# LiHaoy-ux/DQO-MAP

Measured on AMD Instinct MI355X. Metric: mapping iters/sec (fwd+bwd raster) @ 500k Gaussians 1200×680; PSNR vs ref, higher is better.
Workload: dtype f32; 1 GPU; cfg3: surfel room, ONE map of 500000 Gaussians, 1200x680, 8 object ids, SH degree 3, per-object render (object gate) + per-object masked loss (sum over objects of 0.8 L1 colour + 1.0 depth L1 on the object's own mask) + attach loss, raster fwd+bwd + Adam (6 groups); path=fused (hipGraph replays of 4 iterations each); rccl_ranks=1, backend=none (one rank), list_split=0, list_split_backward=0, graph_unroll=4, sync_mode=lazy, selfcheck=skipped, P=500000, P_visible=196562, view=room, adam=exact-sparse, adam_rows_touched=197735, attach_loss_members=49997

## Files before the change

### dqo-map_amd/_dqo_native.py

```python
import ctypes
import os

_HERE = os.path.dirname(os.path.abspath(__file__))
LIB_PATH = os.path.join(_HERE, "lib", "libdqoraster.so")

c_f = ctypes.c_float
c_i32 = ctypes.c_int32
c_vp = ctypes.c_void_p


class DqoRastParams(ctypes.Structure):
    _fields_ = [("P", c_i32), ("D", c_i32), ("M", c_i32), ("W", c_i32), ("H", c_i32), ("prefiltered", c_i32), ("debug", c_i32),
                ("tanfovx", c_f), ("tanfovy", c_f), ("cx", c_f), ("cy", c_f), ("scale_modifier", c_f), ("color_sigma", c_f),
                ("opaque_threshold", c_f), ("depth_threshold", c_f), ("normal_threshold", c_f), ("T_threshold", c_f)]


class DqoRastInputs(ctypes.Structure):
    _fields_ = [(n, c_vp) for n in ("bg", "means3D", "shs", "colors_precomp", "opacities", "scales", "rotations", "cov3D_precomp",
                                    "viewmatrix", "projmatrix", "campos", "tile_mask", "row_flags")]


class DqoRastOutputs(ctypes.Structure):
    _fields_ = [(n, c_vp) for n in ("out_color", "out_depth", "out_hit_color", "out_hit_depth", "out_hit_color_weight",
                                    "out_hit_depth_weight", "out_T", "n_touched", "radii")]
# ... 27 lines not shown

class DqoRastParamGrads(ctypes.Structure):
    _fields_ = [(n, c_vp) for n in ("dL_dfeatures_dc", "dL_dfeatures_rest", "dL_dopacity_raw", "dL_dscaling_raw", "dL_drotation_raw")]


class DqoRastHeader(ctypes.Structure):
    _fields_ = [("num_rendered", ctypes.c_uint32), ("num_tiles", ctypes.c_uint32), ("overflow", ctypes.c_uint32),
                ("max_tile_count", ctypes.c_uint32), ("num_visible", ctypes.c_uint32), ("num_candidates", ctypes.c_uint32),
                ("stage", ctypes.c_uint32), ("reserved", ctypes.c_uint32)]


class DqoProfileEntry(ctypes.Structure):
    _fields_ = [("name", ctypes.c_char * 48), ("total_ms", ctypes.c_double), ("calls", ctypes.c_uint32)]


class DqoAdamStep(ctypes.Structure):
    _fields_ = ([("P", c_i32), ("M", c_i32), ("step", c_i32), ("beta1", c_f), ("beta2", c_f), ("eps", c_f), ("lr_xyz", c_f),
                 ("lr_f_dc", c_f), ("lr_f_rest", c_f), ("lr_opacity", c_f), ("lr_scaling", c_f), ("lr_rotation", c_f)] +
                [(n, c_vp) for n in ("xyz", "shs", "opacity_raw", "scaling_raw", "rotation_raw", "g_means3D", "g_sh", "g_opacity",
                                     "g_scales", "g_rotations", "m_xyz", "m_shs", "m_opacity", "m_scaling", "m_rotation", "v_xyz",
                                     "v_shs", "v_opacity", "v_scaling", "v_rotation", "act_opacity", "act_scales", "act_rotations", "radii", "step_dev", "moment_live",
                                     "attach_mask", "init_xyz", "init_scaling_raw", "init_rotation_raw")] +
                [("attach_count", c_i32), ("attach_partial", c_vp), ("frame_header", c_vp), ("block_ticket", c_vp), ("bias_table", c_vp), ("attach_gains", c_vp),
                 ("row_flags", c_vp), ("confidence", c_vp), ("lr_table", c_vp)])

ROW_FROZEN, ROW_HIDDEN = 1, 2


class DqoAdamTensor(ctypes.Structure):
    _fields_ = [("p", c_vp), ("g", c_vp), ("m", c_vp), ("v", c_vp), ("n", ctypes.c_int64), ("lr", ctypes.c_double)]


EXPORTS = ("dqo_abi_version", "dqo_abi_sizeof", "dqo_last_error", "dqo_profile_enable", "dqo_profile_collect", "dqo_map_activate",
           "dqo_map_loss_workspace_bytes", "dqo_map_loss_fwd_bwd", "dqo_map_ssim_workspace_bytes", "dqo_map_ssim_fwd_bwd", "dqo_map_adam_step", "dqo_adam_multi_dev", "dqo_map_attach_workspace_bytes",
           "dqo_map_attach_loss_fwd_bwd", "dqo_adam_multi", "dqo_accumulate_gaussian_error", "dqo_accumulate_gaussian_confidence", "dqo_rast_geom_bytes", "dqo_rast_image_bytes",
           "dqo_rast_binning_bytes", "dqo_rast_binning_bytes_bucketed",
           "dqo_rast_backward_workspace_bytes", "dqo_rast_forward_prepare", "dqo_rast_read_header", "dqo_rast_forward_render",
           "dqo_rast_forward", "dqo_rast_forward_async", "dqo_rast_backward", "dqo_rast_backward_adam", "dqo_mark_visible", "dqo_knn3_workspace_bytes", "dqo_knn3",
           "dqo_quadric_iou_fwd_bwd", "dqo_quadric_adam", "dqo_tile_count_mask", "dqo_transmission_mask", "dqo_tile_color_error", "dqo_knn3_query_workspace_bytes",
           "dqo_knn3_query", "dqo_knn3_query_within", "dqo_knn3_query_grouped", "dqo_icp_workspace_bytes", "dqo_icp_normal_equations",
           "dqo_attach_pixels", "dqo_attach_decide", "dqo_growth_scales", "dqo_growth_inside", "dqo_error_maps", "dqo_map_history_merge",
           "dqo_rast_forward_prepare_params", "dqo_rast_forward_render_params", "dqo_rast_forward_async_params", "dqo_rast_backward_params",
           "dqo_icp_gauss_newton", "dqo_track_preprocess_workspace_bytes", "dqo_track_preprocess", "dqo_track_pyramid_pixels",
           "dqo_track_pyramid_workspace_bytes", "dqo_track_pyramid", "dqo_track_fill_model_depth", "dqo_track_p2p_workspace_bytes",
           "dqo_track_p2p_loss")

_lib = None
# ... 133 lines not shown
```

### dqo-map_amd/csrc/dqo_adam.h

```cpp
#pragma once
#include "dqo_common.h"

struct AdamArgs {
    int P, M;
    float beta1, beta2, eps, bc2_sqrt;
    float omb1, omb2;
    double beta1_d, beta2_d;
    float step_xyz, step_dc, step_rest, step_opacity, step_scaling, step_rotation;
    float *xyz, *shs, *opacity_raw, *scaling_raw, *rotation_raw;
    const float *g_xyz, *g_shs, *g_opacity, *g_scales, *g_rot;
    float *m_xyz, *m_shs, *m_opacity, *m_scaling, *m_rotation;
    float *v_xyz, *v_shs, *v_opacity, *v_scaling, *v_rotation;
    float *act_opacity, *act_scales, *act_rotations;
    const int32_t* radii;
    uint64_t row_magic;
    const int32_t* step_dev;
    float lr_xyz, lr_dc, lr_rest, lr_opacity, lr_scaling, lr_rotation;
    const uint8_t* attach_mask;
    const float *init_xyz, *init_scaling, *init_rotation;
    float attach_g3, attach_g4;
    float* attach_partial;
    const DqoRastHeader* frame_header;
    int32_t* step_advance;
    int32_t* block_ticket;
    float* bias_table;
    const float* attach_gains;
    const uint8_t* row_flags;
    float* confidence;
    const float* lr_table;
};

static inline double dqo_beta_double(float b) { return (double)(long long)((double)b * 1e7 + 0.5) / 1e7; }

int dqo_adam_args(const DqoAdamStep* st, int blocks, AdamArgs* out, bool* attach);

#ifdef __HIPCC__
constexpr int ADAM_THREADS = 256;

template <typename T>
__device__ __forceinline__ T ldnt(const T* p) {
    return __builtin_nontemporal_load(p);
}
template <typename T>
__device__ __forceinline__ void stnt(T v, T* p) {
    __builtin_nontemporal_store(v, p);
}

__device__ __forceinline__ float adam_wave_red(float v) {
#pragma unroll
    for (int off = 32; off > 0; off >>= 1) v += __shfl_xor(v, off);
    return v;
}

__device__ __forceinline__ void adam1(float& p, float g, float& m, float& v, const AdamArgs& a, float step_size) {
#pragma clang fp contract(off)
    m = m + (g - m) * a.omb1;
    v = v * a.beta2 + a.omb2 * g * g;
    const float denom = sqrtf(v) / a.bc2_sqrt + a.eps;
    p = p - step_size * (m / denom);
}

struct AdamGradGlobal {
    const AdamArgs& a;
    __device__ __forceinline__ float xyz(int, uint32_t, size_t i, bool has_g) const { return a.g_xyz[has_g ? i : 0]; }
    __device__ __forceinline__ float scales(int, uint32_t, size_t i, bool has_g) const { return a.g_scales[has_g ? i : 0]; }
    __device__ __forceinline__ float sh(int, uint32_t, uint32_t ei, uint32_t e0, bool has_g) const { return ldnt(&a.g_shs[has_g ? ei : e0]); }
    __device__ __forceinline__ float opacity(int, uint32_t i, bool has_g) const { return a.g_opacity[has_g ? i : 0u]; }
    __device__ __forceinline__ float4 rot(int, uint32_t i, bool has_g) const { return reinterpret_cast<const float4*>(a.g_rot)[has_g ? i : 0u]; }
    __device__ __forceinline__ bool dc_nonzero(int, uint32_t i, bool has_g) const {
        const size_t e = has_g ? (size_t)i * (size_t)(3 * a.M) : 0;
        const float g0 = ldnt(&a.g_shs[e]), g1 = ldnt(&a.g_shs[e + 1]), g2 = ldnt(&a.g_shs[e + 2]);
        return has_g && (g0 != 0.f || g1 != 0.f || g2 != 0.f);
    }
};

__device__ __forceinline__ void adam_bias_compute(const AdamArgs& a, const int step, float* out ) {
    const double t = (double)step;
    const double bc1 = 1.0 - pow(a.beta1_d, t), bc2 = 1.0 - pow(a.beta2_d, t);
    out[0] = (float)sqrt(bc2);
    float lr[6] = {a.lr_xyz, a.lr_dc, a.lr_rest, a.lr_opacity, a.lr_scaling, a.lr_rotation};
    if (a.lr_table != nullptr) {
#pragma unroll
// ... 62 lines not shown
    const float4 g = has_g ? x.gr_ld : make_float4(0.f, 0.f, 0.f, 0.f);
    const float nrm = fmaxf(sqrtf(q.x * q.x + q.y * q.y + q.z * q.z + q.w * q.w), 1e-12f);
    const float yx = q.x / nrm, yy = q.y / nrm, yz = q.z / nrm, yw = q.w / nrm;
    const float dot = yx * g.x + yy * g.y + yz * g.z + yw * g.w;
    float4 gq = make_float4((g.x - yx * dot) / nrm, (g.y - yy * dot) / nrm, (g.z - yz * dot) / nrm, (g.w - yw * dot) / nrm);
    if (ATTACH) {
        const bool at = ((r >> 30) & 1u) != 0u;
        const float4 q0 = x.q0;
        const float4 d = at ? make_float4(q.x - q0.x, q.y - q0.y, q.z - q0.z, q.w - q0.w) : make_float4(0.f, 0.f, 0.f, 0.f);
        gq.x += a.attach_g4 * d.x, gq.y += a.attach_g4 * d.y, gq.z += a.attach_g4 * d.z, gq.w += a.attach_g4 * d.w;
        att_sum += 0.5f * a.attach_g4 * (d.x * d.x + d.y * d.y + d.z * d.z + d.w * d.w);
    }
    adam1(q.x, gq.x, mq.x, vq.x, a, a.step_rotation);
    adam1(q.y, gq.y, mq.y, vq.y, a, a.step_rotation);
    adam1(q.z, gq.z, mq.z, vq.z, a, a.step_rotation);
    adam1(q.w, gq.w, mq.w, vq.w, a, a.step_rotation);
    reinterpret_cast<float4*>(a.rotation_raw)[i] = q;
    if (a.act_rotations) {
        const float n2 = fmaxf(sqrtf(q.x * q.x + q.y * q.y + q.z * q.z + q.w * q.w), 1e-12f);
        reinterpret_cast<float4*>(a.act_rotations)[i] = make_float4(q.x / n2, q.y / n2, q.z / n2, q.w / n2);
    }
    reinterpret_cast<float4*>(a.m_rotation)[i] = mq;
    reinterpret_cast<float4*>(a.v_rotation)[i] = vq;
    if (a.confidence != nullptr && x.dc_nz) a.confidence[i] = x.conf + 1.0f;
}

template <bool ATTACH, int THREADS, typename GradSrc>
__device__ __forceinline__ float adam_passes(const AdamArgs& a, const uint32_t* s_rows, const int n_rows, const GradSrc& gsrc) {
    const int tid = threadIdx.x;
    float att_sum = 0.f;
    for (int e = tid; e < 3 * n_rows; e += THREADS) {
        const uint32_t k = (uint32_t)e / 3u, j = (uint32_t)e - 3u * k, r = s_rows[k];
        const bool has_g = (r >> 31) != 0u;
        const size_t i = (size_t)(r & 0x3fffffffu) * 3 + j;
        AdamXyzVals x;
        x.p = a.xyz[i], x.m = a.m_xyz[i], x.v = a.v_xyz[i];
        x.ps = a.scaling_raw[i], x.ms = a.m_scaling[i], x.vs = a.v_scaling[i];
        x.gx_ld = gsrc.xyz((int)k, j, i, has_g), x.gs_ld = gsrc.scales((int)k, j, i, has_g);
        x.p0 = x.ps0 = 0.f;
        if (ATTACH) {
            const size_t ai = ((r >> 30) & 1u) ? i : 0;
            x.p0 = a.init_xyz[ai], x.ps0 = a.init_scaling[ai];
        }
        adam_xyz_update<ATTACH>(a, r, i, x, att_sum);
    }
    const uint32_t row = (uint32_t)a.M * 3u;
// ... 186 lines not shown
```

### dqo-map_amd/csrc/map_fused.hip

```cpp
#include "dqo_adam.h"
#include "dqo_common.h"

namespace {

__global__ __launch_bounds__(256) void activate_kernel(int P, const float* __restrict__ opacity_raw, const float* __restrict__ scaling_raw,
                                                       const float* __restrict__ rotation_raw, float* __restrict__ opacity,
                                                       float* __restrict__ scales, float* __restrict__ rotations) {
    const int i = blockIdx.x * blockDim.x + threadIdx.x;
    if (i >= P) return;
    opacity[i] = 1.0f / (1.0f + expf(-opacity_raw[i]));
#pragma unroll
    for (int k = 0; k < 3; k++) scales[3 * i + k] = expf(scaling_raw[3 * i + k]);
    const float4 q = reinterpret_cast<const float4*>(rotation_raw)[i];
    const float n = fmaxf(sqrtf(q.x * q.x + q.y * q.y + q.z * q.z + q.w * q.w), 1e-12f);
    reinterpret_cast<float4*>(rotations)[i] = make_float4(q.x / n, q.y / n, q.z / n, q.w / n);
}

constexpr int LOSS_THREADS = 256;

__device__ __forceinline__ float wave_red(float v) {
#pragma unroll
    for (int off = 32; off > 0; off >>= 1) v += __shfl_xor(v, off);
    return v;
}
// ... 227 lines not shown
        } else {
            const float th0 = acosf(dot), s_th0 = sinf(th0), tht = th0 * t;
            const float s0 = sinf(th0 - tht) / s_th0, s1 = sinf(tht) / s_th0;
            o = make_float4(s0 * v0.x + s1 * v1.x, s0 * v0.y + s1 * v1.y, s0 * v0.z + s1 * v1.z, s0 * v0.w + s1 * v1.w);
        }
        reinterpret_cast<float4*>(rotation)[i] = o;
    }
    const int row = 3 * M;
    const size_t e0 = (size_t)blockIdx.x * HM_THREADS * row;
    const int n = min(HM_THREADS, P - blockIdx.x * HM_THREADS) * row;
    for (int e = threadIdx.x; e < n; e += HM_THREADS) {
        const int r = blockIdx.x * HM_THREADS + e / row;
        if (row_flags != nullptr && (row_flags[r] & DQO_ROW_FROZEN) != 0u) continue;
        shs[e0 + e] = shs0[e0 + e] * w0 + u0 * shs[e0 + e];
    }
}

__global__ void adam_advance_kernel(int32_t* step_dev, const DqoRastHeader* frame_header) {
    if (frame_header != nullptr && frame_header->overflow != 0u) return;
    *step_dev += 1;
}

template <bool SPARSE, bool ATTACH>
__device__ __forceinline__ void adam_block(AdamArgs a, uint8_t* __restrict__ moment_live);

template <bool SPARSE, bool ATTACH>
__global__ __launch_bounds__(ADAM_THREADS) void adam_kernel(const AdamArgs a, uint8_t* __restrict__ moment_live) {
    if (a.frame_header != nullptr && a.frame_header->overflow != 0u) return;
    adam_block<SPARSE, ATTACH>(a, moment_live);
    adam_take_ticket(a);
}

template <bool SPARSE, bool ATTACH>
__device__ __forceinline__ void adam_block(AdamArgs a, uint8_t* __restrict__ moment_live) {
    __shared__ uint32_t s_rows[ADAM_THREADS];
    __shared__ float s_att[ADAM_THREADS / 64];
    __shared__ int s_wave_n[ADAM_THREADS / 64];
    __shared__ float s_ss[7];
    const int tid = threadIdx.x, lane = tid & 63, wave = tid >> 6;
    if (a.step_dev != nullptr && tid == 0) adam_bias_to_lds(a, s_ss);
    const int idx = blockIdx.x * ADAM_THREADS + tid;
    bool hg = false, act = false, att = false;
    if (idx < a.P && !(a.row_flags != nullptr && (a.row_flags[idx] & DQO_ROW_FROZEN) != 0u)) {
        hg = a.radii == nullptr || a.radii[idx] > 0;
        act = !SPARSE || hg || moment_live[idx] != 0;
        if (SPARSE && hg) moment_live[idx] = 1;
        if (ATTACH) att = a.attach_mask[idx] != 0;
    }
    const unsigned long long am = __builtin_amdgcn_ballot_w64(act);
    if (lane == 0) s_wave_n[wave] = (int)__popcll(am);
    __syncthreads();
    if (a.step_dev != nullptr) adam_bias_from_lds(a, s_ss);
    if (ATTACH) adam_attach_gains(a);
    int before = 0, n_rows = 0;
#pragma unroll
    for (int w = 0; w < ADAM_THREADS / 64; w++) {
        const int c = s_wave_n[w];
        before += w < wave ? c : 0;
        n_rows += c;
    }
    if (act) s_rows[before + (int)__popcll(am & ((1ull << lane) - 1ull))] = (uint32_t)idx | (hg ? 0x80000000u : 0u) | (att ? 0x40000000u : 0u);
    __syncthreads();
    if (n_rows == 0) {
        if (ATTACH && a.attach_partial != nullptr && tid == 0) a.attach_partial[blockIdx.x] = 0.f;
        return;
    }
    float att_sum = adam_passes<ATTACH, ADAM_THREADS>(a, s_rows, n_rows, AdamGradGlobal{a});
    if (ATTACH && a.attach_partial != nullptr) {
        att_sum = wave_red(att_sum);
        if (lane == 0) s_att[wave] = att_sum;
// ... 49 lines not shown
    a.step_xyz = (float)((double)st->lr_xyz / bc1);
    a.step_dc = (float)((double)st->lr_f_dc / bc1);
    a.step_rest = (float)((double)st->lr_f_rest / bc1);
    a.step_opacity = (float)((double)st->lr_opacity / bc1);
    a.step_scaling = (float)((double)st->lr_scaling / bc1);
    a.step_rotation = (float)((double)st->lr_rotation / bc1);
    a.xyz = st->xyz, a.shs = st->shs, a.opacity_raw = st->opacity_raw, a.scaling_raw = st->scaling_raw, a.rotation_raw = st->rotation_raw;
    a.g_xyz = st->g_means3D, a.g_shs = st->g_sh, a.g_opacity = st->g_opacity, a.g_scales = st->g_scales, a.g_rot = st->g_rotations;
    a.m_xyz = st->m_xyz, a.m_shs = st->m_shs, a.m_opacity = st->m_opacity, a.m_scaling = st->m_scaling, a.m_rotation = st->m_rotation;
    a.v_xyz = st->v_xyz, a.v_shs = st->v_shs, a.v_opacity = st->v_opacity, a.v_scaling = st->v_scaling, a.v_rotation = st->v_rotation;
    a.act_opacity = st->act_opacity, a.act_scales = st->act_scales, a.act_rotations = st->act_rotations;
    a.radii = st->radii;
    a.step_dev = st->step_dev;
    a.lr_xyz = st->lr_xyz, a.lr_dc = st->lr_f_dc, a.lr_rest = st->lr_f_rest, a.lr_opacity = st->lr_opacity, a.lr_scaling = st->lr_scaling;
    a.lr_rotation = st->lr_rotation;
    a.attach_mask = st->attach_mask, a.init_xyz = st->init_xyz, a.init_scaling = st->init_scaling_raw, a.init_rotation = st->init_rotation_raw;
    a.attach_partial = st->attach_partial, a.frame_header = st->frame_header;
    const bool advance_inside = st->step_dev != nullptr && st->block_ticket != nullptr && blocks > 0;
    a.step_advance = advance_inside ? st->step_dev : nullptr, a.block_ticket = st->block_ticket;
    a.bias_table = (advance_inside && st->step_dev != nullptr) ? st->bias_table : nullptr;
    const bool attach = st->attach_mask != nullptr && (st->attach_count > 0 || st->attach_gains != nullptr);
    a.attach_gains = attach ? st->attach_gains : nullptr;
    a.row_flags = st->row_flags, a.confidence = st->confidence, a.lr_table = st->lr_table;
    DQO_CHECK_ARG(st->lr_table == nullptr || st->step_dev != nullptr, "lr_table is read on the device: it needs step_dev");
    DQO_CHECK_ARG(!attach || (st->init_xyz && st->init_scaling_raw && st->init_rotation_raw), "attach_mask needs the three init_* tensors");
    DQO_CHECK_ARG(st->P < (1 << 30), "P must stay below 2^30");
    a.attach_g3 = (attach && st->attach_count > 0) ? (float)(2000.0 / (3.0 * (double)st->attach_count)) : 0.f;
    a.attach_g4 = (attach && st->attach_count > 0) ? (float)(2000.0 / (4.0 * (double)st->attach_count)) : 0.f;
    DQO_CHECK_ARG(st->M >= 0 && st->M * 3 < 256, "M out of range");
    a.row_magic = st->M > 0 ? ((1ull << 39) + (uint64_t)(3 * st->M) - 1) / (uint64_t)(3 * st->M) : 0ull;
    DQO_CHECK_ARG((int64_t)st->P * (st->M > 0 ? st->M : 1) * 3 < (int64_t)0x7fffffff, "P * M * 3 must stay below 2^31");
    DQO_CHECK_ARG(st->moment_live == nullptr || st->radii != nullptr, "moment_live needs radii");
    *out = a;
    *attach_out = attach;
    return DQO_OK;
}

int dqo_launch_map_adam(const DqoAdamStep* st, hipStream_t s) {
    const int blocks = (st->P + ADAM_THREADS - 1) / ADAM_THREADS;
    AdamArgs a;
    bool attach = false;
    const int rc = dqo_adam_args(st, blocks, &a, &attach);
    if (rc) return rc;
    const bool advance_inside = a.step_advance != nullptr;
    if (blocks > 0) {
        if (st->moment_live != nullptr) {
            if (attach) DQO_LAUNCH("adam_kernel", (adam_kernel<true, true>), dim3(blocks), dim3(ADAM_THREADS), s, a, st->moment_live);
            else DQO_LAUNCH("adam_kernel", (adam_kernel<true, false>), dim3(blocks), dim3(ADAM_THREADS), s, a, st->moment_live);
        } else {
            if (attach) DQO_LAUNCH("adam_kernel", (adam_kernel<false, true>), dim3(blocks), dim3(ADAM_THREADS), s, a, st->moment_live);
            else DQO_LAUNCH("adam_kernel", (adam_kernel<false, false>), dim3(blocks), dim3(ADAM_THREADS), s, a, st->moment_live);
        }
    }
    if (st->step_dev != nullptr && !advance_inside)
        DQO_LAUNCH("adam_advance_kernel", adam_advance_kernel, dim3(1), dim3(1), s, st->step_dev, st->frame_header);
    return DQO_OK;
}

namespace {
constexpr int ADAMM_THREADS = 256, ADAMM_PER_THREAD = 4;
struct AdamMultiArgs {
    float* p[DQO_ADAM_MULTI_MAX];
    const float* g[DQO_ADAM_MULTI_MAX];
    float* m[DQO_ADAM_MULTI_MAX];
    float* v[DQO_ADAM_MULTI_MAX];
    int64_t n[DQO_ADAM_MULTI_MAX];
    float step_size[DQO_ADAM_MULTI_MAX];
    uint32_t first_block[DQO_ADAM_MULTI_MAX + 1];
    int n_tensors;
    float beta1, beta2, omb1, omb2, eps, bc2_sqrt;
    const int32_t* step_dev;
    double beta1_d, beta2_d;
    double lr[DQO_ADAM_MULTI_MAX];
};
// ... 94 lines not shown
```

### dqo-map_amd/csrc/map_fused_tail.hip

```cpp
#include "dqo_adam.h"
#include "dqo_common.h"
#include "dqo_gauss_chain.h"

namespace {

#ifndef DQO_TAIL_THREADS
#define DQO_TAIL_THREADS 128
#endif
constexpr int TAIL_THREADS = DQO_TAIL_THREADS;
constexpr int ROW_MEAN = 0, ROW_W = 3, ROW_RGB = 19, ROW_OP = 22, ROW_SC = 23, ROW_ROT = 26, ROW_STRIDE = 31;

struct AdamGradLds {
    const float* s_g;
    int used3;
    __device__ __forceinline__ float xyz(int k, uint32_t j, size_t, bool) const { return s_g[k * ROW_STRIDE + ROW_MEAN + (int)j]; }
    __device__ __forceinline__ float scales(int k, uint32_t j, size_t, bool) const { return s_g[k * ROW_STRIDE + ROW_SC + (int)j]; }
    __device__ __forceinline__ float sh(int k, uint32_t j, uint32_t, uint32_t, bool) const {
#pragma clang fp contract(off)
        const uint32_t jc = j < (uint32_t)used3 ? j : 0u;
        const uint32_t c = (jc * 171u) >> 9, ch = jc - 3u * c;
        const float g = s_g[k * ROW_STRIDE + ROW_W + (int)c] * s_g[k * ROW_STRIDE + ROW_RGB + (int)ch];
        return j < (uint32_t)used3 ? g : 0.f;
    }
    __device__ __forceinline__ float4 sh4(int k, uint32_t j) const {
        return make_float4(sh(k, j, 0u, 0u, true), sh(k, j + 1u, 0u, 0u, true), sh(k, j + 2u, 0u, 0u, true), sh(k, j + 3u, 0u, 0u, true));
    }
    __device__ __forceinline__ float opacity(int k, uint32_t, bool) const { return s_g[k * ROW_STRIDE + ROW_OP]; }
    __device__ __forceinline__ float4 rot(int k, uint32_t, bool) const {
        const float* r = s_g + k * ROW_STRIDE + ROW_ROT;
        return make_float4(r[0], r[1], r[2], r[3]);
    }
    __device__ __forceinline__ bool dc_nonzero(int k, uint32_t, bool has_g) const {
        return has_g && (sh(k, 0u, 0u, 0u, true) != 0.f || sh(k, 1u, 0u, 0u, true) != 0.f || sh(k, 2u, 0u, 0u, true) != 0.f);
    }
};

#ifndef DQO_TAIL_SH_U
#define DQO_TAIL_SH_U 4
#endif
#ifndef DQO_TAIL_WAVES
#define DQO_TAIL_WAVES 4
#endif
template <bool SPARSE, bool ATTACH>
__global__ __launch_bounds__(TAIL_THREADS, DQO_TAIL_WAVES) void gaussian_tail_kernel(const DqoView v, DqoGeomLayout g, const float* means3D,
                                                                        const float* scales, const float* rotations, const float* shs,
                                                                        const float4* __restrict__ partial,
                                                                        const uint32_t* __restrict__ valid, int64_t capacity, AdamArgs a,
                                                                        uint8_t* __restrict__ moment_live, const uint32_t frame_words,
                                                                        uint32_t* __restrict__ hist, const uint32_t hist_words) {
#pragma clang fp contract(off)
    {
        const uint32_t per = (frame_words + gridDim.x - 1) / gridDim.x;
        const uint32_t z0 = blockIdx.x * per, z1 = min(frame_words, z0 + per);
        for (uint32_t i = z0 + threadIdx.x; i < z1; i += TAIL_THREADS) g.counters[i] = i == 9u ? DQO_CLEARED_STAMP : 0u;
    }
    {
        const uint32_t per = (hist_words + gridDim.x - 1) / gridDim.x;
        const uint32_t z0 = blockIdx.x * per, z1 = min(hist_words, z0 + per);
        for (uint32_t i = z0 + threadIdx.x; i < z1; i += TAIL_THREADS) hist[i] = 0u;
    }
    const uint32_t ovf_ld = a.frame_header != nullptr ? a.frame_header->overflow : 0u;
    int step_ld = 0;
    float tb[8] = {0.f, 0.f, 0.f, 0.f, 0.f, 0.f, 0.f, 0.f};
    if (a.step_dev != nullptr) {
        step_ld = *a.step_dev;
        if (a.bias_table != nullptr) {
#pragma unroll
            for (int i = 0; i < 8; i++) tb[i] = a.bias_table[i];
        }
    }
    if (ATTACH) adam_attach_gains(a);
    __shared__ float4 s_buf[(TAIL_THREADS * ROW_STRIDE * 4 + 15) / 16];
    float4* const s_rec = s_buf;
    float* const s_g = reinterpret_cast<float*>(s_buf);
    static_assert(sizeof(float4) * TAIL_THREADS * 4 <= sizeof(s_buf), "the slot staging must fit the buffer");
    __shared__ uint32_t s_rows[TAIL_THREADS];
    __shared__ uint32_t s_lohi[2 * (TAIL_THREADS / 64)];
    __shared__ int s_wave_n[TAIL_THREADS / 64];
    __shared__ float s_att[TAIL_THREADS / 64];
    const int tid = threadIdx.x, lane = tid & 63, wave = tid >> 6;
    const int idx = dqo_spread_index(blockIdx.x * TAIL_THREADS + tid, v.P);
    const bool in_range = idx < v.P;

    uint2 rc = make_uint2(0u, 0u);
    uint32_t base = 0, cnt = 0;
    bool live_m = false, att = false, trained = in_range;
    if (in_range) {
        rc = g.rect16[idx];
        cnt = g.tiles_touched[idx];
        base = g.slot_base[idx];
        if (SPARSE) live_m = moment_live[idx] != 0;
        if (ATTACH) att = a.attach_mask[idx] != 0;
        if (a.row_flags != nullptr) trained = (a.row_flags[idx] & DQO_ROW_FROZEN) == 0u;
    }
    float view[16], proj[16];
#pragma unroll
    for (int i = 0; i < 16; i++) {
        view[i] = __int_as_float(__builtin_amdgcn_readfirstlane(__float_as_int(v.view[i])));
        proj[i] = __int_as_float(__builtin_amdgcn_readfirstlane(__float_as_int(v.proj[i])));
    }
    if (ovf_ld != 0u) return;
    if (a.step_dev != nullptr) {
        float ss[7];
        if (a.bias_table != nullptr && __float_as_int(tb[7]) == step_ld) {
#pragma unroll
            for (int i = 0; i < 7; i++) ss[i] = tb[i];
        } else {
            adam_bias_compute(a, step_ld, ss);
        }
        adam_bias_from_lds(a, ss);
    }
    if (!trained) cnt = 0u, live_m = false, att = false;
    const bool visible = trained && ((rc.x >> 16) > (rc.x & 0xffffu)) && ((rc.y >> 16) > (rc.y & 0xffffu));
    const bool act = trained && (!SPARSE || visible || live_m);
    if (SPARSE && visible) moment_live[idx] = 1;
    const unsigned long long am = __builtin_amdgcn_ballot_w64(act);
    const uint32_t w_lo = ~dqo_wave_max_u32(cnt ? ~base : 0u, lane), w_hi = dqo_wave_max_u32(cnt ? base + cnt : 0u, lane);
    if (lane == 0) s_wave_n[wave] = (int)__popcll(am), s_lohi[2 * wave] = w_lo, s_lohi[2 * wave + 1] = w_hi;
    __syncthreads();
    int before = 0, n_rows = 0;
    uint32_t lo = 0xffffffffu, hi_all = 0u;
#pragma unroll
    for (int w = 0; w < TAIL_THREADS / 64; w++) {
        const int c = s_wave_n[w];
        before += w < wave ? c : 0;
        n_rows += c;
        lo = min(lo, s_lohi[2 * w]), hi_all = max(hi_all, s_lohi[2 * w + 1]);
    }
    const int my_row = before + (int)__popcll(am & ((1ull << lane) - 1ull));
    if (act) s_rows[my_row] = (uint32_t)idx | (visible ? 0x80000000u : 0u) | (att ? 0x40000000u : 0u);
    const uint32_t hi = (uint32_t)min((int64_t)hi_all, capacity);

    DqoChainIn ci;
#pragma unroll
    for (int i = 0; i < 9; i++) ci.dd[i] = 0.f;
    ci.cop = make_float4(0.f, 0.f, 0.f, 0.f);
    ci.mx = ci.my = ci.mz = ci.sx = ci.sy = ci.sz = 0.f;
    ci.qt = make_float4(1.f, 0.f, 0.f, 0.f);
    ci.n_np = ci.pc = make_float4(0.f, 0.f, 0.f, 0.f);
    ci.cl = 0;
    if (visible) {
        ci.cop = g.conic_opacity[idx];
        ci.mx = means3D[3 * idx], ci.my = means3D[3 * idx + 1], ci.mz = means3D[3 * idx + 2];
        ci.sx = scales[3 * idx], ci.sy = scales[3 * idx + 1], ci.sz = scales[3 * idx + 2];
        ci.qt = reinterpret_cast<const float4*>(rotations)[idx];
        ci.n_np = g.normal_c[idx], ci.pc = g.point_c[idx], ci.cl = g.clamped[idx];
        const float4* ddp = g.drgb_dir + 3 * (size_t)idx;
        const float4 d0 = ddp[0], d1 = ddp[1], d2 = ddp[2];
        ci.dd[0] = d0.x, ci.dd[1] = d0.y, ci.dd[2] = d0.z, ci.dd[3] = d1.x, ci.dd[4] = d1.y, ci.dd[5] = d1.z;
        ci.dd[6] = d2.x, ci.dd[7] = d2.y, ci.dd[8] = d2.z;
    }

    float4 a0 = make_float4(0.f, 0.f, 0.f, 0.f), a1 = a0, a2 = a0, a3 = a0;
    if (lo < hi) {
        const float4 z = make_float4(0.f, 0.f, 0.f, 0.f);
        for (uint32_t c0 = lo; c0 < hi; c0 += TAIL_THREADS) {
            const uint32_t slot = c0 + tid;
            if (slot < hi) {
                const uint32_t vw = valid[slot];
                const float4* p = partial + (size_t)slot * 16;
                float4 r[4][4];
#pragma unroll
                for (int q = 0; q < 4; q++) {
                    const float4* src = ((vw >> (8 * q)) & 0xffu) ? p + 4 * q : partial;
#pragma unroll
                    for (int i = 0; i < 4; i++) r[q][i] = src[i];
                }
                float4 m0 = z, m1 = z, m2 = z, m3 = z;
#pragma unroll
                for (int q = 0; q < 4; q++) {
                    const uint32_t bq = (vw >> (8 * q)) & 0xffu;
                    if (bq) {
                        const float4 r0 = r[q][0], r1 = r[q][1], r2 = r[q][2], r3 = r[q][3];
                        m0.x += r0.x, m0.y += r0.y, m0.z += r0.z, m0.w += r0.w;
                        m1.x += r1.x, m1.y += r1.y, m1.z += r1.z, m1.w += r1.w;
                        m2.x += r2.x;
                        if (bq & 2u) {
                            m2.y += r2.y, m2.z += r2.z, m2.w += r2.w;
                            m3.x += r3.x, m3.y += r3.y;
                        }
                    }
                }
                s_rec[tid * 4] = m0, s_rec[tid * 4 + 1] = m1, s_rec[tid * 4 + 2] = m2, s_rec[tid * 4 + 3] = m3;
            }
            __syncthreads();
            const uint32_t k0 = max(base, c0), k1 = min(base + cnt, min(c0 + (uint32_t)TAIL_THREADS, hi));
            for (uint32_t k = k0; k < k1; k++) {
                const float4 r0 = s_rec[(k - c0) * 4], r1 = s_rec[(k - c0) * 4 + 1], r2 = s_rec[(k - c0) * 4 + 2], r3 = s_rec[(k - c0) * 4 + 3];
                a0.x += r0.x, a0.y += r0.y, a0.z += r0.z, a0.w += r0.w;
                a1.x += r1.x, a1.y += r1.y, a1.z += r1.z, a1.w += r1.w;
                a2.x += r2.x, a2.y += r2.y, a2.z += r2.z, a2.w += r2.w;
                a3.x += r3.x, a3.y += r3.y, a3.z += r3.z, a3.w += r3.w;
            }
            __syncthreads();
        }
    }
    if (n_rows == 0) {
        if (ATTACH && a.attach_partial != nullptr && tid == 0) a.attach_partial[blockIdx.x] = 0.f;
        adam_take_ticket(a);
        return;
    }

    if (visible) {
        ci.a[0] = a0.x, ci.a[1] = a0.y, ci.a[2] = a0.z, ci.a[3] = a0.w;
        ci.a[4] = a1.x, ci.a[5] = a1.y, ci.a[6] = a1.z, ci.a[7] = a1.w;
        ci.a[8] = a2.x, ci.a[9] = a2.y, ci.a[10] = a2.z, ci.a[11] = a2.w;
        ci.a[12] = a3.x, ci.a[13] = a3.y, ci.a[14] = a3.z, ci.a[15] = a3.w;
        if (cnt == 0u) ci.cop = make_float4(0.f, 0.f, 0.f, 0.f);
        DqoChainOut co;
        dqo_gauss_chain(v, view, proj, ci, true, co);
        float* row = s_g + my_row * ROW_STRIDE;
        row[ROW_MEAN] = co.mean_g[0], row[ROW_MEAN + 1] = co.mean_g[1], row[ROW_MEAN + 2] = co.mean_g[2];
#pragma unroll
        for (int k = 0; k < 16; k++) row[ROW_W + k] = co.w[k];
        row[ROW_RGB] = co.dRGB[0], row[ROW_RGB + 1] = co.dRGB[1], row[ROW_RGB + 2] = co.dRGB[2];
        row[ROW_OP] = co.dop;
        row[ROW_SC] = co.dsc[0], row[ROW_SC + 1] = co.dsc[1], row[ROW_SC + 2] = co.dsc[2];
        row[ROW_ROT] = co.rot_g[0], row[ROW_ROT + 1] = co.rot_g[1], row[ROW_ROT + 2] = co.rot_g[2], row[ROW_ROT + 3] = co.rot_g[3];
    }
    __syncthreads();
    const int used = (v.D + 1) * (v.D + 1);
    const bool vec4 = v.M == 16 && ((reinterpret_cast<uintptr_t>(a.shs) | reinterpret_cast<uintptr_t>(a.m_shs) |
                                     reinterpret_cast<uintptr_t>(a.v_shs)) & 15u) == 0u;
    float att_sum;
    if (vec4) att_sum = adam_passes_tail<ATTACH, TAIL_THREADS, true, DQO_TAIL_SH_U>(a, s_rows, n_rows, AdamGradLds{s_g, 3 * used});
    else att_sum = adam_passes<ATTACH, TAIL_THREADS>(a, s_rows, n_rows, AdamGradLds{s_g, 3 * used});
    if (ATTACH && a.attach_partial != nullptr) {
        att_sum = adam_wave_red(att_sum);
        if (TAIL_THREADS == 64) {
            if (lane == 0) a.attach_partial[blockIdx.x] = att_sum;
        } else {
// ... 45 lines not shown
                   in->rotations, in->shs, reinterpret_cast<const float4*>(recs), reinterpret_cast<const uint32_t*>(valid), cap, gr, frame_words,
                   hist, hist_words, dL_drest);
        return DQO_OK;
    }
    DQO_LAUNCH("gaussian_rows_kernel", gaussian_rows_kernel, dim3(blocks), dim3(TAIL_THREADS), s, v, g, in->means3D, in->scales, in->rotations,
               in->shs, reinterpret_cast<const float4*>(recs), reinterpret_cast<const uint32_t*>(valid), cap, gr, frame_words, hist, hist_words);
    return DQO_OK;
}

int dqo_launch_blend_backward(const DqoView& v, const DqoGeomLayout& g, const DqoImageLayout& img, const DqoBinLayout& bin, int T,
                              const float* dL_dcolor, const float* dL_ddepth, DqoGradRec* recs, uint8_t* valid, int64_t capacity,
                              const DqoTapDev& tap, const DqoGateDev& gate, int list_split, hipStream_t s);
int dqo_launch_adam_advance(int32_t* step_dev, const DqoRastHeader* frame_header, hipStream_t s);

int dqo_launch_backward_adam(const DqoRastParams* p, const DqoRastInputs* in, const DqoRastCtx* ctx, const float* dL_dcolor,
                             const float* dL_ddepth, const DqoAdamStep* st, void* ws, hipStream_t s) {
    if (p->P <= 0) return DQO_OK;
    const DqoView v = dqo_make_view(p, in);
    DqoGeomLayout g = dqo_geom_layout(ctx->geom, p->P);
    DqoImageLayout img = dqo_image_layout(ctx->image, p->W, p->H);
    DqoBinLayout bin = dqo_bin_layout(ctx->binning, ctx->inst_capacity,
                                      dqo_list_cap(ctx->inst_capacity, p->W, p->H, ctx->tile_bucket_capacity), ctx->tile_bucket_capacity);
    const int T = v.gx * v.gy;
    const int64_t cap = (int64_t)ctx->inst_capacity;
    DqoGradRec* recs = (DqoGradRec*)ws;
    uint8_t* valid = reinterpret_cast<uint8_t*>(bin.rec_valid);
    const int blocks = dqo_spread_blocks(p->P) * (256 / TAIL_THREADS);
    AdamArgs a;
    bool attach = false;
    int rc = dqo_adam_args(st, blocks, &a, &attach);
    if (rc) return rc;
    a.frame_header = g.header;
    rc = dqo_launch_blend_backward(v, g, img, bin, T, dL_dcolor, dL_ddepth, recs, valid, cap, dqo_tap_dev(ctx->loss_tap),
                                   dqo_gate_dev(ctx->object_gate), dqo_list_split(ctx), s);
    if (rc) return rc;
    const float4* partial = reinterpret_cast<const float4*>(recs);
    const uint32_t* vw = reinterpret_cast<const uint32_t*>(valid);
    const uint32_t frame_words = (uint32_t)dqo_frame_scalar_words(ctx);
    const uint32_t hist_words = (uint32_t)((img.tile_flag + T) - img.tile_count);
#define DQO_TAIL(SP, AT)                                                                                                              \
    DQO_LAUNCH("gaussian_tail_kernel", (gaussian_tail_kernel<SP, AT>), dim3(blocks), dim3(TAIL_THREADS), s, v, g, in->means3D, in->scales, \
               in->rotations, in->shs, partial, vw, cap, a, st->moment_live, frame_words, img.tile_count, hist_words)
    if (st->moment_live != nullptr) {
        if (attach) DQO_TAIL(true, true);
        else DQO_TAIL(true, false);
    } else {
        if (attach) DQO_TAIL(false, true);
        else DQO_TAIL(false, false);
    }
#undef DQO_TAIL
    if (st->step_dev != nullptr && a.step_advance == nullptr) return dqo_launch_adam_advance(st->step_dev, g.header, s);
    return DQO_OK;
}
```

### dqo-map_amd/dqo_harness/fused_mapping.py

```python
import collections
import ctypes
import os
import threading

import numpy as np
import torch

import _dqo_native as N
import diff_gaussian_rasterization_depth as dgr
from dqo_harness import mapping


def _normalised_settings(st, device):
    def fix(t, name, n):
        if not torch.is_tensor(t):
            raise RuntimeError(f"raster settings: {name} must be a tensor")
        if t.dtype != torch.float32:
            raise RuntimeError(f"expected scalar type Float but found {t.dtype} ({name})")
        if not t.is_cuda:
            raise RuntimeError("libdqoraster operators need GPU (ROCm) tensors; there is no CPU path.")
        if t.numel() != n:
            raise RuntimeError(f"raster settings: {name} must have {n} elements")
        return t.to(device).contiguous()
    return st._replace(bg=fix(st.bg, "bg", 3), viewmatrix=fix(st.viewmatrix, "viewmatrix", 16), projmatrix=fix(st.projmatrix, "projmatrix", 16),
# ... 692 lines not shown
                              binning_bytes=g.binning.numel(), image=g.img.data_ptr(), image_bytes=g.img.numel(), inst_capacity=g.cap,
                              tile_bucket_capacity=g.bucket)
        g.ls_fwd, g.ls_bwd = self.pick_list_split_pair(opt["list_split"], g.tile_mask, st, longest)
        g.cctx.list_split = g.ls_fwd
        loss_tap = opt["loss_tap"] and not (g.mask is None and self.ssim_weight != 0)
        if loss_tap:
            g.grad_scale = torch.zeros((2,), dtype=torch.float32, device=self.device)
            g.tap = N.DqoLossTap(gt_color=N.ptr(g.gt_color), gt_depth=N.ptr(g.gt_depth), render_mask=N.ptr(g.mask),
                                 out_color=g.out[0].data_ptr(), out_depth=g.out[1].data_ptr(), color_weight=self.color_weight,
                                 depth_weight=self.depth_weight, add_depth_thres=self.add_depth_thres, loss_out=N.ptr(self.loss),
                                 grad_scale=g.grad_scale.data_ptr(),
                                 per_object=1 if (self.per_object_loss and self.gaussian_object is not None) else 0)
            g.cctx.loss_tap = ctypes.addressof(g.tap)
        if self.gaussian_object is not None:
            g.gate = N.DqoObjectGate(gaussian_object=N.ptr(self.gaussian_object), pixel_object=N.ptr(g.pixel_object),
                                     tile_objects=N.ptr(g.tile_objects))
            g.cctx.object_gate = ctypes.addressof(g.gate)
            if self.per_object_loss and not loss_tap:
                raise RuntimeError("FusedMapper.capture: the per-object loss is computed by the loss tap (loss_tap=True)")
        gr = [g.grads[k].data_ptr() for k in ("means3D", "sh", "opacity", "scales", "rot")]
        g.cgrads = N.DqoRastGrads(dL_dmeans3D=gr[0], dL_dsh=gr[1], dL_dcolors=None, dL_dopacity=gr[2], dL_dscales=gr[3],
                                  dL_drotations=gr[4], dL_dcov3D=None, dL_dmeans2D=None, skip_culled_rows=1)
        g.adam = self._adam_step_args(gr, radii=g.out[8].data_ptr(), frame_header=g.geom.data_ptr(), step_dev=g.step_dev)

    def _warm_up_and_record(self, g, reuse_probe):
        self._step_dev.fill_(self.step_count + 1)
        self._expected_step = self.step_count + 1
        side = torch.cuda.Stream(device=self.device)
        side.wait_stream(torch.cuda.current_stream())
        with torch.cuda.stream(side):
            self._static_iteration()
        torch.cuda.current_stream().wait_stream(side)
        if not self.graph_overflowed():
            self.step_count += 1
        elif reuse_probe:
            return False
        g.cctx.keep_tile_order = 1 if (g.bucket > 0 and g.options["keep_tile_order"]) else 0
        g.cctx.frame_prezeroed = 1 if g.fused_tail else 0
        g.graph = torch.cuda.CUDAGraph()
        g.unroll = max(1, int(g.options["unroll"]))
        with torch.cuda.graph(g.graph, capture_error_mode="thread_local"):
            for _ in range(g.unroll):
                self._static_iteration()
        g.run_unroll = max(1, int(g.options["run_unroll"]))
        if g.run_unroll > 1:
            g.run_graph = torch.cuda.CUDAGraph()
# ... 376 lines not shown
```

### include/dqo_raster.h

```cpp
#ifndef DQO_RASTER_H_
#define DQO_RASTER_H_

#include <stddef.h>
#include <stdint.h>

#ifdef __cplusplus
extern "C" {
#endif

#define DQO_ABI_VERSION 5

typedef enum DqoStatus {
    DQO_OK = 0,
    DQO_ERR_INVALID_ARG = -1,
    DQO_ERR_WORKSPACE = -2,
    DQO_ERR_LAUNCH = -3,
    DQO_ERR_OVERFLOW = -4
} DqoStatus;

typedef struct DqoRastParams {
    int32_t P;
    int32_t D;
    int32_t M;
    int32_t W, H;
// ... 272 lines not shown
    int32_t P, M;
    int32_t step;
    float beta1, beta2, eps;
    float lr_xyz, lr_f_dc, lr_f_rest, lr_opacity, lr_scaling, lr_rotation;
    float *xyz, *shs, *opacity_raw, *scaling_raw, *rotation_raw;
    const float *g_means3D, *g_sh, *g_opacity, *g_scales, *g_rotations;
    float *m_xyz, *m_shs, *m_opacity, *m_scaling, *m_rotation;
    float *v_xyz, *v_shs, *v_opacity, *v_scaling, *v_rotation;
    float *act_opacity, *act_scales, *act_rotations;
    const int32_t* radii;
    int32_t* step_dev;
    uint8_t* moment_live;
    const uint8_t* attach_mask;
    const float *init_xyz, *init_scaling_raw, *init_rotation_raw;
    int32_t attach_count;
    float* attach_partial;
    const DqoRastHeader* frame_header;
    int32_t* block_ticket;
    float* bias_table;
    const float* attach_gains;
    const uint8_t* row_flags;
    float* confidence;
    const float* lr_table;
} DqoAdamStep;
int dqo_map_adam_step(const DqoAdamStep*, void* hipStream);

int dqo_map_history_merge(int32_t P, int32_t M, float max_weight, int32_t first_row, const uint8_t* row_flags, const float* conf0,
                          const float* conf, const float* xyz0, const float* shs0, const float* scaling0, const float* rot0_unit, float* xyz,
                          float* shs, float* scaling_raw, float* rotation_raw, void* hipStream);

int dqo_rast_backward_adam(const DqoRastParams*, const DqoRastInputs*, const DqoRastCtx*, const float* dL_dout_color,
                           const float* dL_dout_depth, const DqoAdamStep* step, void* workspace, size_t workspace_bytes,
                           void* hipStream);

#ifdef __cplusplus
}
#endif
#endif
```

Before: 2331 iter/s.

## Treat Gaussians without valid backward records as gradient-free in sparse Adam

Sparse Adam and the fused tail now mark a row as having a gradient only when at least one of its per-tile backward records is valid, not merely when it is visible. Visible rows whose records are all empty, for example ones gated out by the per-object mask, skip moment updates unless they already have live moments or are attach members. moment_live is now set only after an actual update. The tail kernel builds its row list after the record scan instead of before it. The aim is to cut the number of rows touched by Adam, at the cost of an extra scan of record-valid words and a changed sync structure in the tail.

```diff
diff --git a/dqo-map_amd/_dqo_native.py b/dqo-map_amd/_dqo_native.py
--- a/dqo-map_amd/_dqo_native.py
+++ b/dqo-map_amd/_dqo_native.py
@@ -73,7 +73,7 @@
                                      "v_shs", "v_opacity", "v_scaling", "v_rotation", "act_opacity", "act_scales", "act_rotations", "radii", "step_dev", "moment_live",
                                      "attach_mask", "init_xyz", "init_scaling_raw", "init_rotation_raw")] +
                 [("attach_count", c_i32), ("attach_partial", c_vp), ("frame_header", c_vp), ("block_ticket", c_vp), ("bias_table", c_vp), ("attach_gains", c_vp),
-                 ("row_flags", c_vp), ("confidence", c_vp), ("lr_table", c_vp)])
+                 ("row_flags", c_vp), ("confidence", c_vp), ("lr_table", c_vp), ("record_ctx", c_vp), ("record_W", c_i32), ("record_H", c_i32)])
 
 ROW_FROZEN, ROW_HIDDEN = 1, 2
 
diff --git a/dqo-map_amd/csrc/dqo_adam.h b/dqo-map_amd/csrc/dqo_adam.h
--- a/dqo-map_amd/csrc/dqo_adam.h
+++ b/dqo-map_amd/csrc/dqo_adam.h
@@ -28,6 +28,9 @@
     const uint8_t* row_flags;
     float* confidence;
     const float* lr_table;
+    const uint32_t *rec_count, *rec_base, *rec_valid;
+    int64_t rec_capacity;
+    uint8_t* moment_live;
 };
 
 static inline double dqo_beta_double(float b) { return (double)(long long)((double)b * 1e7 + 0.5) / 1e7; }
@@ -58,6 +61,14 @@
     v = v * a.beta2 + a.omb2 * g * g;
     const float denom = sqrtf(v) / a.bc2_sqrt + a.eps;
     p = p - step_size * (m / denom);
+}
+
+__device__ __forceinline__ bool adam_has_record(const AdamArgs& a, const int idx) {
+    const uint32_t base = a.rec_base[idx];
+    const uint32_t end = (uint32_t)min((int64_t)base + (int64_t)a.rec_count[idx], a.rec_capacity);
+    uint32_t any = 0u;
+    for (uint32_t s = base; s < end; s++) any |= a.rec_valid[s];
+    return any != 0u;
 }
 
 struct AdamGradGlobal {
@@ -166,6 +177,7 @@
     }
     reinterpret_cast<float4*>(a.m_rotation)[i] = mq;
     reinterpret_cast<float4*>(a.v_rotation)[i] = vq;
+    if (a.moment_live != nullptr) a.moment_live[i] = 1;
     if (a.confidence != nullptr && x.dc_nz) a.confidence[i] = x.conf + 1.0f;
 }
 
diff --git a/dqo-map_amd/csrc/map_fused.hip b/dqo-map_amd/csrc/map_fused.hip
--- a/dqo-map_amd/csrc/map_fused.hip
+++ b/dqo-map_amd/csrc/map_fused.hip
@@ -273,17 +273,17 @@
 }
 
 template <bool SPARSE, bool ATTACH>
-__device__ __forceinline__ void adam_block(AdamArgs a, uint8_t* __restrict__ moment_live);
+__device__ __forceinline__ void adam_block(AdamArgs a);
 
 template <bool SPARSE, bool ATTACH>
-__global__ __launch_bounds__(ADAM_THREADS) void adam_kernel(const AdamArgs a, uint8_t* __restrict__ moment_live) {
+__global__ __launch_bounds__(ADAM_THREADS) void adam_kernel(const AdamArgs a) {
     if (a.frame_header != nullptr && a.frame_header->overflow != 0u) return;
-    adam_block<SPARSE, ATTACH>(a, moment_live);
+    adam_block<SPARSE, ATTACH>(a);
     adam_take_ticket(a);
 }
 
 template <bool SPARSE, bool ATTACH>
-__device__ __forceinline__ void adam_block(AdamArgs a, uint8_t* __restrict__ moment_live) {
+__device__ __forceinline__ void adam_block(AdamArgs a) {
     __shared__ uint32_t s_rows[ADAM_THREADS];
     __shared__ float s_att[ADAM_THREADS / 64];
     __shared__ int s_wave_n[ADAM_THREADS / 64];
@@ -293,10 +293,12 @@
     const int idx = blockIdx.x * ADAM_THREADS + tid;
     bool hg = false, act = false, att = false;
     if (idx < a.P && !(a.row_flags != nullptr && (a.row_flags[idx] & DQO_ROW_FROZEN) != 0u)) {
-        hg = a.radii == nullptr || a.radii[idx] > 0;
-        act = !SPARSE || hg || moment_live[idx] != 0;
-        if (SPARSE && hg) moment_live[idx] = 1;
+        const bool visible = a.radii == nullptr || a.radii[idx] > 0;
         if (ATTACH) att = a.attach_mask[idx] != 0;
+        hg = visible;
+        if (SPARSE && visible && a.rec_valid != nullptr) hg = adam_has_record(a, idx);
+        const bool live_m = SPARSE && a.moment_live[idx] != 0;
+        act = !SPARSE || hg || live_m || (visible && att);
     }
     const unsigned long long am = __builtin_amdgcn_ballot_w64(act);
     if (lane == 0) s_wave_n[wave] = (int)__popcll(am);
@@ -392,6 +394,17 @@
     const bool attach = st->attach_mask != nullptr && (st->attach_count > 0 || st->attach_gains != nullptr);
     a.attach_gains = attach ? st->attach_gains : nullptr;
     a.row_flags = st->row_flags, a.confidence = st->confidence, a.lr_table = st->lr_table;
+    a.rec_count = a.rec_base = a.rec_valid = nullptr, a.rec_capacity = 0;
+    a.moment_live = st->moment_live;
+    if (st->record_ctx != nullptr && st->moment_live != nullptr) {
+        const DqoRastCtx* c = st->record_ctx;
+        DQO_CHECK_ARG(c->geom != nullptr && c->binning != nullptr && st->record_W > 0 && st->record_H > 0, "record_ctx needs its buffers and record_W / record_H");
+        const DqoGeomLayout g = dqo_geom_layout(c->geom, st->P);
+        const DqoBinLayout bin = dqo_bin_layout(c->binning, c->inst_capacity,
+                                                dqo_list_cap(c->inst_capacity, st->record_W, st->record_H, c->tile_bucket_capacity),
+                                                c->tile_bucket_capacity);
+        a.rec_count = g.tiles_touched, a.rec_base = g.slot_base, a.rec_valid = bin.rec_valid, a.rec_capacity = (int64_t)c->inst_capacity;
+    }
     DQO_CHECK_ARG(st->lr_table == nullptr || st->step_dev != nullptr, "lr_table is read on the device: it needs step_dev");
     DQO_CHECK_ARG(!attach || (st->init_xyz && st->init_scaling_raw && st->init_rotation_raw), "attach_mask needs the three init_* tensors");
     DQO_CHECK_ARG(st->P < (1 << 30), "P must stay below 2^30");
@@ -415,11 +428,11 @@
     const bool advance_inside = a.step_advance != nullptr;
     if (blocks > 0) {
         if (st->moment_live != nullptr) {
-            if (attach) DQO_LAUNCH("adam_kernel", (adam_kernel<true, true>), dim3(blocks), dim3(ADAM_THREADS), s, a, st->moment_live);
-            else DQO_LAUNCH("adam_kernel", (adam_kernel<true, false>), dim3(blocks), dim3(ADAM_THREADS), s, a, st->moment_live);
+            if (attach) DQO_LAUNCH("adam_kernel", (adam_kernel<true, true>), dim3(blocks), dim3(ADAM_THREADS), s, a);
+            else DQO_LAUNCH("adam_kernel", (adam_kernel<true, false>), dim3(blocks), dim3(ADAM_THREADS), s, a);
         } else {
-            if (attach) DQO_LAUNCH("adam_kernel", (adam_kernel<false, true>), dim3(blocks), dim3(ADAM_THREADS), s, a, st->moment_live);
-            else DQO_LAUNCH("adam_kernel", (adam_kernel<false, false>), dim3(blocks), dim3(ADAM_THREADS), s, a, st->moment_live);
+            if (attach) DQO_LAUNCH("adam_kernel", (adam_kernel<false, true>), dim3(blocks), dim3(ADAM_THREADS), s, a);
+            else DQO_LAUNCH("adam_kernel", (adam_kernel<false, false>), dim3(blocks), dim3(ADAM_THREADS), s, a);
         }
     }
     if (st->step_dev != nullptr && !advance_inside)
diff --git a/dqo-map_amd/csrc/map_fused_tail.hip b/dqo-map_amd/csrc/map_fused_tail.hip
--- a/dqo-map_amd/csrc/map_fused_tail.hip
+++ b/dqo-map_amd/csrc/map_fused_tail.hip
@@ -46,7 +46,7 @@
                                                                         const float* scales, const float* rotations, const float* shs,
                                                                         const float4* __restrict__ partial,
                                                                         const uint32_t* __restrict__ valid, int64_t capacity, AdamArgs a,
-                                                                        uint8_t* __restrict__ moment_live, const uint32_t frame_words,
+                                                                        const uint32_t frame_words,
                                                                         uint32_t* __restrict__ hist, const uint32_t hist_words) {
 #pragma clang fp contract(off)
     {
@@ -89,7 +89,7 @@
         rc = g.rect16[idx];
         cnt = g.tiles_touched[idx];
         base = g.slot_base[idx];
-        if (SPARSE) live_m = moment_live[idx] != 0;
+        if (SPARSE) live_m = a.moment_live[idx] != 0;
         if (ATTACH) att = a.attach_mask[idx] != 0;
         if (a.row_flags != nullptr) trained = (a.row_flags[idx] & DQO_ROW_FROZEN) == 0u;
     }
@@ -112,23 +112,33 @@
     }
     if (!trained) cnt = 0u, live_m = false, att = false;
     const bool visible = trained && ((rc.x >> 16) > (rc.x & 0xffffu)) && ((rc.y >> 16) > (rc.y & 0xffffu));
-    const bool act = trained && (!SPARSE || visible || live_m);
-    if (SPARSE && visible) moment_live[idx] = 1;
-    const unsigned long long am = __builtin_amdgcn_ballot_w64(act);
     const uint32_t w_lo = ~dqo_wave_max_u32(cnt ? ~base : 0u, lane), w_hi = dqo_wave_max_u32(cnt ? base + cnt : 0u, lane);
-    if (lane == 0) s_wave_n[wave] = (int)__popcll(am), s_lohi[2 * wave] = w_lo, s_lohi[2 * wave + 1] = w_hi;
-    __syncthreads();
-    int before = 0, n_rows = 0;
+    if (lane == 0) s_lohi[2 * wave] = w_lo, s_lohi[2 * wave + 1] = w_hi;
+    int my_row = 0, n_rows = 0;
+    auto list_rows = [&](const bool act, const uint32_t word) {
+        const unsigned long long am = __builtin_amdgcn_ballot_w64(act);
+        if (lane == 0) s_wave_n[wave] = (int)__popcll(am);
+        __syncthreads();
+        int before = 0;
+#pragma unroll
+        for (int w = 0; w < TAIL_THREADS / 64; w++) {
+            const int c = s_wave_n[w];
+            before += w < wave ? c : 0;
+            n_rows += c;
+        }
+        my_row = before + (int)__popcll(am & ((1ull << lane) - 1ull));
+        if (act) s_rows[my_row] = word;
+    };
+    constexpr uint32_t CNT_ATT = 0x20000000u, CNT_LIVE = 0x40000000u, REC_ANY = 0x80000000u, CNT_MASK = 0x1fffffffu;
+    if (SPARSE) {
+        cnt |= (att ? CNT_ATT : 0u) | (live_m ? CNT_LIVE : 0u);
+        __syncthreads();
+    } else {
+        list_rows(trained, (uint32_t)idx | (visible ? 0x80000000u : 0u) | (att ? 0x40000000u : 0u));
+    }
     uint32_t lo = 0xffffffffu, hi_all = 0u;
 #pragma unroll
-    for (int w = 0; w < TAIL_THREADS / 64; w++) {
-        const int c = s_wave_n[w];
-        before += w < wave ? c : 0;
-        n_rows += c;
-        lo = min(lo, s_lohi[2 * w]), hi_all = max(hi_all, s_lohi[2 * w + 1]);
-    }
-    const int my_row = before + (int)__popcll(am & ((1ull << lane) - 1ull));
-    if (act) s_rows[my_row] = (uint32_t)idx | (visible ? 0x80000000u : 0u) | (att ? 0x40000000u : 0u);
+    for (int w = 0; w < TAIL_THREADS / 64; w++) lo = min(lo, s_lohi[2 * w]), hi_all = max(hi_all, s_lohi[2 * w + 1]);
     const uint32_t hi = (uint32_t)min((int64_t)hi_all, capacity);
 
     DqoChainIn ci;
@@ -139,7 +149,7 @@
     ci.qt = make_float4(1.f, 0.f, 0.f, 0.f);
     ci.n_np = ci.pc = make_float4(0.f, 0.f, 0.f, 0.f);
     ci.cl = 0;
-    if (visible) {
+    if (visible && (!SPARSE || (cnt & CNT_MASK) != 0u)) {
         ci.cop = g.conic_opacity[idx];
         ci.mx = means3D[3 * idx], ci.my = means3D[3 * idx + 1], ci.mz = means3D[3 * idx + 2];
         ci.sx = scales[3 * idx], ci.sy = scales[3 * idx + 1], ci.sz = scales[3 * idx + 2];
@@ -155,6 +165,7 @@
     if (lo < hi) {
         const float4 z = make_float4(0.f, 0.f, 0.f, 0.f);
         for (uint32_t c0 = lo; c0 < hi; c0 += TAIL_THREADS) {
+            if (c0 != lo) __syncthreads();
             const uint32_t slot = c0 + tid;
             if (slot < hi) {
                 const uint32_t vw = valid[slot];
@@ -181,19 +192,28 @@
                         }
                     }
                 }
+                m3.w = __uint_as_float(vw);
                 s_rec[tid * 4] = m0, s_rec[tid * 4 + 1] = m1, s_rec[tid * 4 + 2] = m2, s_rec[tid * 4 + 3] = m3;
             }
             __syncthreads();
-            const uint32_t k0 = max(base, c0), k1 = min(base + cnt, min(c0 + (uint32_t)TAIL_THREADS, hi));
+            const uint32_t k0 = max(base, c0), k1 = min(base + (cnt & CNT_MASK), min(c0 + (uint32_t)TAIL_THREADS, hi));
             for (uint32_t k = k0; k < k1; k++) {
                 const float4 r0 = s_rec[(k - c0) * 4], r1 = s_rec[(k - c0) * 4 + 1], r2 = s_rec[(k - c0) * 4 + 2], r3 = s_rec[(k - c0) * 4 + 3];
                 a0.x += r0.x, a0.y += r0.y, a0.z += r0.z, a0.w += r0.w;
                 a1.x += r1.x, a1.y += r1.y, a1.z += r1.z, a1.w += r1.w;
                 a2.x += r2.x, a2.y += r2.y, a2.z += r2.z, a2.w += r2.w;
-                a3.x += r3.x, a3.y += r3.y, a3.z += r3.z, a3.w += r3.w;
+                a3.x += r3.x, a3.y += r3.y;
+                cnt |= __float_as_uint(r3.w) != 0u ? REC_ANY : 0u;
             }
-            __syncthreads();
-        }
+        }
+    }
+    const bool has_grad = visible && (!SPARSE || (cnt & REC_ANY) != 0u);
+    if (SPARSE) {
+        const bool act = has_grad || (cnt & CNT_LIVE) != 0u || (visible && (cnt & CNT_ATT) != 0u);
+        list_rows(act, (uint32_t)dqo_spread_index(blockIdx.x * TAIL_THREADS + tid, v.P) | (has_grad ? 0x80000000u : 0u) |
+                           ((cnt & CNT_ATT) ? 0x40000000u : 0u));
+    } else if (lo < hi) {
+        __syncthreads();
     }
     if (n_rows == 0) {
         if (ATTACH && a.attach_partial != nullptr && tid == 0) a.attach_partial[blockIdx.x] = 0.f;
@@ -201,12 +221,12 @@
         return;
     }
 
-    if (visible) {
+    if (has_grad) {
         ci.a[0] = a0.x, ci.a[1] = a0.y, ci.a[2] = a0.z, ci.a[3] = a0.w;
         ci.a[4] = a1.x, ci.a[5] = a1.y, ci.a[6] = a1.z, ci.a[7] = a1.w;
         ci.a[8] = a2.x, ci.a[9] = a2.y, ci.a[10] = a2.z, ci.a[11] = a2.w;
         ci.a[12] = a3.x, ci.a[13] = a3.y, ci.a[14] = a3.z, ci.a[15] = a3.w;
-        if (cnt == 0u) ci.cop = make_float4(0.f, 0.f, 0.f, 0.f);
+        if ((cnt & CNT_MASK) == 0u) ci.cop = make_float4(0.f, 0.f, 0.f, 0.f);
         DqoChainOut co;
         dqo_gauss_chain(v, view, proj, ci, true, co);
         float* row = s_g + my_row * ROW_STRIDE;
@@ -298,6 +318,7 @@
     DqoBinLayout bin = dqo_bin_layout(ctx->binning, ctx->inst_capacity,
                                       dqo_list_cap(ctx->inst_capacity, p->W, p->H, ctx->tile_bucket_capacity), ctx->tile_bucket_capacity);
     const int T = v.gx * v.gy;
+    DQO_CHECK_ARG(T < (1 << 29), "more than 2^29 tiles");
     const int64_t cap = (int64_t)ctx->inst_capacity;
     DqoGradRec* recs = (DqoGradRec*)ws;
     uint8_t* valid = reinterpret_cast<uint8_t*>(bin.rec_valid);
@@ -306,6 +327,7 @@
     bool attach = false;
     int rc = dqo_adam_args(st, blocks, &a, &attach);
     if (rc) return rc;
+    a.rec_count = a.rec_base = a.rec_valid = nullptr;
     a.frame_header = g.header;
     rc = dqo_launch_blend_backward(v, g, img, bin, T, dL_dcolor, dL_ddepth, recs, valid, cap, dqo_tap_dev(ctx->loss_tap),
                                    dqo_gate_dev(ctx->object_gate), dqo_list_split(ctx), s);
@@ -316,7 +338,7 @@
     const uint32_t hist_words = (uint32_t)((img.tile_flag + T) - img.tile_count);
 #define DQO_TAIL(SP, AT)                                                                                                              \
     DQO_LAUNCH("gaussian_tail_kernel", (gaussian_tail_kernel<SP, AT>), dim3(blocks), dim3(TAIL_THREADS), s, v, g, in->means3D, in->scales, \
-               in->rotations, in->shs, partial, vw, cap, a, st->moment_live, frame_words, img.tile_count, hist_words)
+               in->rotations, in->shs, partial, vw, cap, a, frame_words, img.tile_count, hist_words)
     if (st->moment_live != nullptr) {
         if (attach) DQO_TAIL(true, true);
         else DQO_TAIL(true, false);
diff --git a/dqo-map_amd/dqo_harness/fused_mapping.py b/dqo-map_amd/dqo_harness/fused_mapping.py
--- a/dqo-map_amd/dqo_harness/fused_mapping.py
+++ b/dqo-map_amd/dqo_harness/fused_mapping.py
@@ -738,6 +738,8 @@
         g.cgrads = N.DqoRastGrads(dL_dmeans3D=gr[0], dL_dsh=gr[1], dL_dcolors=None, dL_dopacity=gr[2], dL_dscales=gr[3],
                                   dL_drotations=gr[4], dL_dcov3D=None, dL_dmeans2D=None, skip_culled_rows=1)
         g.adam = self._adam_step_args(gr, radii=g.out[8].data_ptr(), frame_header=g.geom.data_ptr(), step_dev=g.step_dev)
+        g.adam.record_ctx = ctypes.addressof(g.cctx)
+        g.adam.record_W, g.adam.record_H = int(st.image_width), int(st.image_height)
 
     def _warm_up_and_record(self, g, reuse_probe):
         self._step_dev.fill_(self.step_count + 1)
diff --git a/include/dqo_raster.h b/include/dqo_raster.h
--- a/include/dqo_raster.h
+++ b/include/dqo_raster.h
@@ -318,6 +318,8 @@
     const uint8_t* row_flags;
     float* confidence;
     const float* lr_table;
+    const DqoRastCtx* record_ctx;
+    int32_t record_W, record_H;
 } DqoAdamStep;
 int dqo_map_adam_step(const DqoAdamStep*, void* hipStream);
 
```

After: 2380 iter/s (median of 6 runs). +2.1%, better.
